# nyx-space/nyx

Measured on NVIDIA H100. Metric: trajectory-steps/sec (ensemble), higher is better.
Workload: dtype f64

## Files before the change

### nyx_b200/csrc/nyxb_tx.cu

```cuda
#include <algorithm>
#include <cmath>
#include <cstring>
#include <numeric>

#include "nyxb_tx.h"

#ifndef TX_MINB
#define TX_MINB 2
#endif

#ifndef NYXB_TX_TT
#define NYXB_TX_TT 1
#endif

namespace {
constexpr int TT = NYXB_TX_TT;
constexpr int NL = 32 * TT;
constexpr int HW = 3 * TT;
constexpr unsigned FULL = 0xffffffffu;

enum { TXF_H = 0, TXF_ERR, TXF_CR, TXF_CD, TXF_PM, TXF_DRY, TXF_EXTRA, TXF_SRPA, TXF_DRAGA, TXF_EVPREV, TXF_COUNT };
enum { TXI_EPOCH = 0, TXI_STEP, TXI_PREV_STEP, TXI_DET_STEP, TXI_NSTEPS, TXI_NREJ, TXI_NRHS, TXI_COUNT };
enum { TXW_FLAGS = 0, TXW_STATUS, TXW_RC, TXW_ATT, TXW_EVCNT, TXW_ACC, TXW_RCST, TXW_COUNT };
enum { F_FIXED = 1, F_PREVFIXED = 2, F_RETRY = 4, F_LAST = 8, F_DONE = 16, F_BACK = 32, F_VALID = 64 };

struct TxLayout {
    unsigned blob, ctx0, ctx_stride;
    unsigned wk, part, as, ysp, kst, nxt, er, ycur, rot, rn, f64, i64, i32;
    unsigned total;
};
__host__ __device__ inline TxLayout tx_layout(unsigned blob_bytes, int P, int N, int nctx) {
    (void)N;
    TxLayout L;
    L.blob = 0;
    L.ctx0 = (blob_bytes + 127u) & ~127u;
    unsigned o = 0;
    L.wk = o; o += 2u * (P == 16 ? 20u : 6u * (unsigned)P + 4u) * NL * 8;
    L.part = o; o += 2u * (unsigned)P * 4 * NL * 8;
    L.as = o; o += 2u * 18u * NL * 8;
    L.ysp = o; o += 2u * 3u * NL * 8;
    L.kst = o; o += NYXB_MAX_STAGES * 6 * NL * 8;
    L.nxt = o; o += 6 * NL * 8;
    L.er = o; o += 6 * NL * 8;
    L.ycur = o; o += 6 * NL * 8;
    L.rot = o; o += 6 * NL * 8;
    L.rn = o; o += 2u * 9u * NL * 8;
    L.f64 = o; o += TXF_COUNT * NL * 8;
    L.i64 = o; o += TXI_COUNT * NL * 8;
    L.i32 = o; o += TXW_COUNT * NL * 4;
    L.ctx_stride = (o + 127u) & ~127u;
    L.total = L.ctx0 + (unsigned)nctx * L.ctx_stride;
    return L;
}

struct TxSm {
    double *wk, *part, *as, *ysp, *kst, *nxt, *er, *ycur, *rot, *rn, *f64;
    long long* i64;
    int* i32;
};
__device__ __forceinline__ TxSm tx_views(unsigned char* smem, const TxLayout& L, int ctx, int N) {
    (void)N;
    unsigned char* b = smem + L.ctx0 + (unsigned)ctx * L.ctx_stride;
    TxSm sm;
    sm.wk = reinterpret_cast<double*>(b + L.wk); sm.part = reinterpret_cast<double*>(b + L.part);
    sm.as = reinterpret_cast<double*>(b + L.as); sm.ysp = reinterpret_cast<double*>(b + L.ysp);
    sm.kst = reinterpret_cast<double*>(b + L.kst); sm.nxt = reinterpret_cast<double*>(b + L.nxt);
    sm.er = reinterpret_cast<double*>(b + L.er); sm.ycur = reinterpret_cast<double*>(b + L.ycur);
    sm.rot = reinterpret_cast<double*>(b + L.rot); sm.rn = reinterpret_cast<double*>(b + L.rn);
    sm.f64 = reinterpret_cast<double*>(b + L.f64); sm.i64 = reinterpret_cast<long long*>(b + L.i64);
    sm.i32 = reinterpret_cast<int*>(b + L.i32);
    return sm;
}

__device__ __forceinline__ void nb_sync(int id, int count) { asm volatile("bar.sync %0, %1;" ::"r"(id), "r"(count) : "memory"); }
__device__ __forceinline__ void nb_arrive(int id, int count) { asm volatile("bar.arrive %0, %1;" ::"r"(id), "r"(count) : "memory"); }

__device__ __forceinline__ unsigned smem_u32(const void* p) { return (unsigned)__cvta_generic_to_shared(p); }
__device__ __forceinline__ void tx_mbar_init(unsigned long long* bar, unsigned count) {
    asm volatile("mbarrier.init.shared::cta.b64 [%0], %1;" ::"r"(smem_u32(bar)), "r"(count));
    asm volatile("fence.mbarrier_init.release.cluster;" ::: "memory");
}
__device__ __forceinline__ void tx_mbar_expect(unsigned long long* bar, unsigned bytes) {
    asm volatile("mbarrier.arrive.expect_tx.shared::cta.b64 _, [%0], %1;" ::"r"(smem_u32(bar)), "r"(bytes) : "memory");
}
__device__ __forceinline__ void tx_bulk_g2s(void* dst, const void* src, unsigned bytes, unsigned long long* bar) {
    asm volatile("cp.async.bulk.shared::cluster.global.mbarrier::complete_tx::bytes [%0], [%1], %2, [%3];"
                 ::"r"(smem_u32(dst)), "l"(src), "r"(bytes), "r"(smem_u32(bar)) : "memory");
}
__device__ __forceinline__ void tx_mbar_wait(unsigned long long* bar, unsigned parity) {
    asm volatile(
        "{\n"
        ".reg .pred p;\n"
        "TX_WAIT_LOOP:\n"
        "mbarrier.try_wait.parity.shared::cta.b64 p, [%0], %1;\n"
        "@p bra TX_WAIT_DONE;\n"
        "bra TX_WAIT_LOOP;\n"
        "TX_WAIT_DONE:\n"
        "}\n" ::"r"(smem_u32(bar)), "r"(parity) : "memory");
}

__device__ __forceinline__ void tx_mbar_arrive(unsigned long long* bar) {
// ... 273 lines not shown
        sm.i64[TXI_NSTEPS * NL + lane] = 0;
        sm.i64[TXI_NREJ * NL + lane] = 0;
        sm.i64[TXI_NRHS * NL + lane] = 0;
        sm.i32[TXW_FLAGS * NL + lane] = fl;
        sm.i32[TXW_STATUS * NL + lane] = 0;
        sm.i32[TXW_RC * NL + lane] = rc;
        sm.i32[TXW_ATT * NL + lane] = 1;
        sm.i32[TXW_EVCNT * NL + lane] = 0;
        sm.f64[TXF_EVPREV * NL + lane] = 0.0;
        if (sink.ev_kind)
            sm.f64[TXF_EVPREV * NL + lane] = event_eval(sink.ev_kind, sink.ev_value, state[tr], state[n + tr], state[2 * n + tr],
                                                        state[3 * n + tr], state[4 * n + tr], state[5 * n + tr]);
        if (valid && sink.cap > 0) sink.epoch[tr] = ep0;
    } else {
        const int pf = __ldcg(q.ws_flags + tr);
        const nyxb_details* dp = q.details + tr;
        sm.f64[TXF_CR * NL + lane] = __ldcg(out_state + 6 * n + tr);
        sm.f64[TXF_CD * NL + lane] = __ldcg(out_state + 7 * n + tr);
        sm.f64[TXF_PM * NL + lane] = __ldcg(out_state + 8 * n + tr);
        sm.f64[TXF_H * NL + lane] = __ldcg(q.ws_f64 + tr);
        sm.f64[TXF_EVPREV * NL + lane] = __ldcg(q.ws_f64 + n + tr);
        sm.f64[TXF_ERR * NL + lane] = __ldcg(&dp->error);
        sm.i64[TXI_EPOCH * NL + lane] = __ldcg(out_epoch + tr);
        const long long step_ns = __ldcg(q.ws_step + tr);
        sm.i64[TXI_STEP * NL + lane] = step_ns;
        sm.i64[TXI_PREV_STEP * NL + lane] = step_ns;
        sm.i64[TXI_DET_STEP * NL + lane] = __ldcg((const long long*)&dp->step_ns);
        sm.i64[TXI_NSTEPS * NL + lane] = __ldcg((const long long*)&dp->n_steps);
        sm.i64[TXI_NREJ * NL + lane] = __ldcg((const long long*)&dp->n_rejected);
        sm.i64[TXI_NRHS * NL + lane] = __ldcg((const long long*)&dp->n_rhs);
        sm.i32[TXW_ATT * NL + lane] = __ldcg(&dp->attempts);
        int fl = (pf & (F_FIXED | F_RETRY | F_DONE)) | (valid ? F_VALID : 0) | (duration < 0 ? F_BACK : 0);
        if (!valid) fl |= F_DONE;
        sm.i32[TXW_FLAGS * NL + lane] = fl;
        sm.i32[TXW_STATUS * NL + lane] = (pf & 8) ? NYXB_WARN_MAX_ATTEMPTS : 0;
        sm.i32[TXW_RC * NL + lane] = (pf >> 8) & 0xff;
        sm.i32[TXW_EVCNT * NL + lane] = sink.ev_kind ? __ldcg(sink.ev_crossings + tr) : 0;
    }
}

__device__ __noinline__ void tx_park_ctl(const DevSink& sink, const DevTxQueue& q, TxSm sm, int lane, size_t n, size_t tr,
                                         long long* step_io, double* out_state, long long* out_epoch, int* out_status) {
    const int fl = sm.i32[TXW_FLAGS * NL + lane];
    if (!(fl & F_VALID)) return;
    const int rc = sm.i32[TXW_RC * NL + lane], st = sm.i32[TXW_STATUS * NL + lane];
    out_state[6 * n + tr] = sm.f64[TXF_CR * NL + lane];
    out_state[7 * n + tr] = sm.f64[TXF_CD * NL + lane];
    out_state[8 * n + tr] = sm.f64[TXF_PM * NL + lane];
    out_epoch[tr] = sm.i64[TXI_EPOCH * NL + lane];
    const long long step_ns = sm.i64[TXI_STEP * NL + lane];
    q.ws_step[tr] = step_ns;
    q.ws_f64[tr] = sm.f64[TXF_H * NL + lane];
    q.ws_f64[n + tr] = sm.f64[TXF_EVPREV * NL + lane];
    q.ws_flags[tr] = (fl & (F_FIXED | F_RETRY | F_DONE)) | ((st & NYXB_WARN_MAX_ATTEMPTS) ? 8 : 0) | (rc << 8);
    nyxb_details d;
    d.step_ns = sm.i64[TXI_DET_STEP * NL + lane];
    d.error = sm.f64[TXF_ERR * NL + lane];
    d.attempts = sm.i32[TXW_ATT * NL + lane];
    d._pad = 0;
    d.n_steps = sm.i64[TXI_NSTEPS * NL + lane];
    d.n_rejected = sm.i64[TXI_NREJ * NL + lane];
    d.n_rhs = sm.i64[TXI_NRHS * NL + lane];
    q.details[tr] = d;
    int rc_out = rc;
    if (sink.ev_kind) {
        const int cnt = sm.i32[TXW_EVCNT * NL + lane];
        sink.ev_crossings[tr] = cnt;
        if (rc == 0 && cnt < sink.ev_trigger) rc_out = NYXB_ERR_EVENT_NOT_FOUND;
    }
    out_status[tr] = (st & NYXB_WARN_MAX_ATTEMPTS) | rc_out;
    if (step_io) step_io[tr] = step_ns;
    if (sink.cap > 0) sink.count[tr] = (d.n_steps + 1 < sink.cap) ? d.n_steps + 1 : sink.cap;
}

enum { AS_R = 0, AS_S = 9, AS_T, AS_U, AS_K0, AS_K1, AS_FAC, AS_P0, AS_P1, AS_P2, AS_COUNT };
enum { WK_UB = 0, WK_R2, WK_POW };
template <int P> struct TxWk {
    static constexpr bool ALL = (P != 16);
    static constexpr int E = 2 * P;
    static constexpr int COUNT = ALL ? WK_POW + 3 * E + 2 : WK_POW + 18;
    static constexpr int ZR = WK_POW, ZI = WK_POW + E + 1, RH = WK_POW + 2 * E + 1;
};

template <int P>
__device__ __forceinline__ void tx_prologue(const DevSetup& S, const TxSm& sm, int lane, int par, int j, const double* ysp, long long t_ns) {
    const DevGrav& gv = S.grav;
    const double* rn = sm.rn + par * 9 * NL + lane;
    const double p0 = ysp[lane], p1 = ysp[NL + lane], p2 = ysp[2 * NL + lane];
    double y0 = p0, y1 = p1, y2 = p2;
    double ir_c = 0.0;
    if (S.grav_body >= 0) {
        ir_c = rsqrt(fma(y2, y2, fma(y1, y1, y0 * y0)));
        tx_field_offset(S, t_ns, y0, y1, y2);
    }
    const double rb0 = fma(rn[2 * NL], y2, fma(rn[1 * NL], y1, rn[0] * y0));
    const double rb1 = fma(rn[5 * NL], y2, fma(rn[4 * NL], y1, rn[3 * NL] * y0));
    const double rb2 = fma(rn[8 * NL], y2, fma(rn[7 * NL], y1, rn[6 * NL] * y0));
    const double inv_r = rsqrt(fma(rb2, rb2, fma(rb1, rb1, rb0 * rb0)));
    if (S.grav_body < 0) ir_c = inv_r;
    const double rho = gv.r_eq * inv_r;
    const double s_ = rb0 * inv_r, t_ = rb1 * inv_r, u_ = rb2 * inv_r;
    double* wk = sm.wk + par * TxWk<P>::COUNT * NL + lane;
    if (j == 0) {
        wk[WK_UB * NL] = u_ * rho; wk[WK_R2 * NL] = rho * rho;
        double* as = sm.as + par * AS_COUNT * NL + lane;
#pragma unroll
        for (int k = 0; k < 9; ++k) as[(AS_R + k) * NL] = rn[k * NL];
        as[AS_S * NL] = s_; as[AS_T * NL] = t_; as[AS_U * NL] = u_;
        const double K0 = (gv.mu * gv.inv_r_eq) * inv_r;
        as[AS_K0 * NL] = K0; as[AS_K1 * NL] = K0 * rho;
        as[AS_FAC * NL] = -S.mu_central * ir_c * ir_c * ir_c;
        as[AS_P0 * NL] = p0; as[AS_P1 * NL] = p1; as[AS_P2 * NL] = p2;
        if constexpr (!TxWk<P>::ALL) {
            double zr = s_, zi = t_, rp = rho;
#pragma unroll
            for (int k = 0; k < 6; ++k) {
                wk[(WK_POW + 3 * k) * NL] = zr; wk[(WK_POW + 3 * k + 1) * NL] = zi; wk[(WK_POW + 3 * k + 2) * NL] = rp;
                const double nr = fma(zr, zr, -(zi * zi));
                zi = 2.0 * zr * zi; zr = nr; rp *= rp;
            }
        }
    } else if constexpr (TxWk<P>::ALL) {
        constexpr int E = TxWk<P>::E;
        static_assert(E > 8 && E <= 24, "published powers");
        double* wr = wk + TxWk<P>::ZR * NL;
        double* wi = wk + TxWk<P>::ZI * NL;
        double zr[9], zi[9];
        zr[1] = s_; zi[1] = t_;
#pragma unroll
        for (int lo = 1; lo < 8; lo *= 2) {
#pragma unroll
            for (int k = 1; k <= lo; ++k) {
                zr[lo + k] = fma(zr[lo], zr[k], -(zi[lo] * zi[k]));
                zi[lo + k] = fma(zr[lo], zi[k], zi[lo] * zr[k]);
            }
        }
        if (j == 1) {
            wr[0] = 1.0; wi[0] = 0.0;
#pragma unroll
            for (int k = 1; k <= 8; ++k) { wr[k * NL] = zr[k]; wi[k * NL] = zi[k]; }
            double rp[9];
            rp[1] = rho;
#pragma unroll
            for (int lo = 1; lo < 8; lo *= 2) {
#pragma unroll
                for (int k = 1; k <= lo; ++k) rp[lo + k] = rp[lo] * rp[k];
            }
            double* wp = wk + TxWk<P>::RH * NL;
            const double r16 = rp[8] * rp[8];
#pragma unroll
            for (int k = 1; k <= 8; ++k) {
                wp[k * NL] = rp[k];
                if (8 + k <= E) wp[(8 + k) * NL] = (k == 8) ? r16 : rp[8] * rp[k];
                if (16 + k <= E) wp[(16 + k) * NL] = r16 * rp[k];
            }
        } else {
            const double z16r = fma(zr[8], zr[8], -(zi[8] * zi[8])), z16i = 2.0 * zr[8] * zi[8];
#pragma unroll
            for (int k = 1; k <= 8; ++k) {
                if (8 + k <= E) {
                    wr[(8 + k) * NL] = (k == 8) ? z16r : fma(zr[8], zr[k], -(zi[8] * zi[k]));
                    wi[(8 + k) * NL] = (k == 8) ? z16i : fma(zr[8], zi[k], zi[8] * zr[k]);
                }
                if (16 + k <= E) {
                    wr[(16 + k) * NL] = fma(z16r, zr[k], -(z16i * zi[k]));
                    wi[(16 + k) * NL] = fma(z16r, zi[k], z16i * zr[k]);
                }
            }
        }
    }
}

struct TxRotBase { double sa, ca, sd, cd, sw, cw; };
__device__ __forceinline__ void tx_dcm(const DevRotation& rot, const TxRotBase& b, long long off_ns, double (&R)[9]) {
    if (rot.kind == 0) {
        R[0] = 1; R[1] = 0; R[2] = 0; R[3] = 0; R[4] = 1; R[5] = 0; R[6] = 0; R[7] = 0; R[8] = 1;
        return;
    }
    const double dt_s = (double)off_ns * 1e-9;
    const double da = rot.ra_dot * dt_s, dd = rot.dec_dot * dt_s, dw = rot.wdot * dt_s;
    const double sa = fma(b.ca, da, b.sa), ca = fma(-b.sa, da, b.ca);
    const double sd = fma(b.cd, dd, b.sd), cd = fma(-b.sd, dd, b.cd);
    double sdl, cdl;
    if (fabs(dw) < 0.02) {
        const double z = dw * dw;
        sdl = dw * fma(z, fma(z, 1.0 / 120.0, -1.0 / 6.0), 1.0);
        cdl = fma(z, fma(z, fma(z, -1.0 / 720.0, 1.0 / 24.0), -0.5), 1.0);
    } else {
        det_sincos(dw, sdl, cdl);
    }
    const double sw = fma(b.sw, cdl, b.cw * sdl), cw = fma(b.cw, cdl, -(b.sw * sdl));
    const double b00 = -sa, b01 = ca;
    const double b10 = -(sd * ca), b11 = -(sd * sa), b12 = cd;
    R[0] = fma(cw, b00, sw * b10); R[1] = fma(cw, b01, sw * b11); R[2] = sw * b12;
    R[3] = fma(cw, b10, -(sw * b00)); R[4] = fma(cw, b11, -(sw * b01)); R[5] = cw * b12;
    R[6] = cd * ca; R[7] = cd * sa; R[8] = sd;
}

__device__ __forceinline__ TxRotBase tx_rot_base(const DevRotation& rot, long long epoch) {
    TxRotBase b;
    const double t_s = dur_to_seconds(epoch);
    const double d = t_s / 86400.0;
    const double Tc = d / 36525.0;
    det_sincos((rot.ra0 + rot.ra1 * Tc) * NYXB_DEG2RAD, b.sa, b.ca);
    det_sincos((rot.dec0 + rot.dec1 * Tc) * NYXB_DEG2RAD, b.sd, b.cd);
    det_sincos(fmod(rot.w0 + rot.w1 * d, 360.0) * NYXB_DEG2RAD, b.sw, b.cw);
    return b;
}
__device__ __forceinline__ void tx_rot_store(double* rot, int lane, const TxRotBase& b) {
    rot[lane] = b.sa; rot[NL + lane] = b.ca; rot[2 * NL + lane] = b.sd; rot[3 * NL + lane] = b.cd; rot[4 * NL + lane] = b.sw;
    rot[5 * NL + lane] = b.cw;
}

template <int W, int NB>
__device__ __forceinline__ void tx_start_powers(const double* wk, double& zar, double& zai, double& pa, double& zbr, double& zbi, double& pb) {
    const double rho = wk[(WK_POW + 2) * NL];
    bool fa = true, fb = true;
    zar = 1.0; zai = 0.0; zbr = 1.0; zbi = 0.0; pa = rho; pb = rho;
#pragma unroll
    for (int k = 0; k < NB; ++k) {
        const double br = wk[(WK_POW + 3 * k) * NL], bi = wk[(WK_POW + 3 * k + 1) * NL], bp = wk[(WK_POW + 3 * k + 2) * NL];
        if ((W >> k) & 1) {
            if (fa) { zar = br; zai = bi; fa = false; }
            else { const double nr = fma(zar, br, -(zai * bi)); zai = fma(zar, bi, zai * br); zar = nr; }
            pa *= bp;
        } else {
            if (fb) { zbr = br; zbi = bi; fb = false; }
            else { const double nr = fma(zbr, br, -(zbi * bi)); zbi = fma(zbr, bi, zbi * br); zbr = nr; }
            pb *= bp;
        }
    }
}

template <int P, int NCTX>
__global__ void __launch_bounds__((P + HW * NCTX) * 32, 1)
nyxb_k_tx(const __grid_constant__ DevSetup S, const __grid_constant__ DevTx Tx, const __grid_constant__ DevTxQueue q, size_t n,
          const double* __restrict__ state, const double* __restrict__ consts, const long long* __restrict__ epoch0,
          long long end_epoch, long long* step_io, double* out_state, long long* out_epoch, int* out_status, const DevSink sink,
          unsigned blob_bytes, unsigned off_recK, unsigned off_seed, unsigned off_sched) {
    static_assert(P <= NYXB_TX_MAXP && NCTX >= 1 && NCTX <= 2, "walker positions / set contexts");
    extern __shared__ __align__(128) unsigned char smem[];
    __shared__ __align__(8) unsigned long long tma_bar;
    __shared__ __align__(8) unsigned long long ready_bar[NCTX][2];
    __shared__ int s_set[NCTX], s_fresh[NCTX], s_exit[NCTX], s_done_half[NCTX][TT], s_slice_end[NCTX];
    __shared__ __align__(8) unsigned long long kick_bar;
    const int tid = threadIdx.x, lane = tid & 31, w = tid >> 5;
#ifdef NYXB_TX_TRACE
    int tr_n = 0;
#endif
    constexpr int NPOW = 6;
    static_assert(P == 8 || P == 10 || P == 16, "walker positions");
    static_assert(TT == 1 || NCTX == 1, "sets of 64 trajectories: one set context per CTA");
    constexpr int NT_RW = (P + HW) * 32;
    constexpr int NT_HB = HW * 32;
    constexpr int BAR_PER_CTX = 5;
    const int N = S.grav.N;
    const int stages = S.tb.stages;
    const TxLayout L = tx_layout(blob_bytes, P, N, NCTX);
    const double2* recA = reinterpret_cast<const double2*>(smem + L.blob);
    const double* recK = reinterpret_cast<const double*>(smem + L.blob + off_recK);
    const double* colseed = reinterpret_cast<const double*>(smem + L.blob + off_seed);
    const int* sched = reinterpret_cast<const int*>(smem + L.blob + off_sched);

    if (tid == 0) {
        tx_mbar_init(&tma_bar, 1);
#pragma unroll
        tx_mbar_init(&kick_bar, 1);
#pragma unroll
        for (int c = 0; c < NCTX; ++c) {
            s_exit[c] = 0;
            tx_mbar_init(&ready_bar[c][0], NT_HB);
            tx_mbar_init(&ready_bar[c][1], NT_HB);
        }
    }
    __syncthreads();
    if (tid == 0) {
        tx_mbar_expect(&tma_bar, blob_bytes);
        tx_bulk_g2s(smem + L.blob, Tx.recA, blob_bytes, &tma_bar);
    }
    tx_mbar_wait(&tma_bar, 0);
    __syncthreads();

    if (w < P) {
        const int pos = (P == 8) ? ((0x23571046u >> (4 * w)) & 0xfu) : w;
        const int* my = sched + pos * (2 + 2 * Tx.kmax);
        const int rec_off = my[0], ncol = my[1];
        unsigned active = (1u << NCTX) - 1u;
        unsigned phases = 0;
        const unsigned ready0 = smem_u32(&ready_bar[0][0]);
        int stage0 = 0, stage1 = 0, pref = 0;
        while (active) {
            {
                int c = -1, par = 0;
                TX_TRACE(TR_POLL, 0, 0);
                for (;;) {
#pragma unroll
                    for (int k = 0; k < NCTX; ++k) {
                        const int cc = (pref + k) % NCTX;
                        if (c >= 0 || !((active >> cc) & 1u)) continue;
                        const int pp = (cc == 0 ? stage0 : stage1) & 1;
                        const bool ok = tx_mbar_test(ready0 + 8u * (unsigned)(2 * cc + pp), (phases >> (2 * cc + pp)) & 1u);
                        if (__all_sync(FULL, ok)) { c = cc; par = pp; }
                    }
                    if (c >= 0) break;
                    __nanosleep(20);
                }
                phases ^= 1u << (2 * c + par);
                const int st = (c == 0) ? stage0 : stage1;
                if (st == 0 && *(volatile int*)&s_exit[c]) { active &= ~(1u << c); continue; }
                const int stn = (st + 1 == stages) ? 0 : st + 1;
                if (c == 0) stage0 = stn; else stage1 = stn;
                pref = (c + 1) % NCTX;
                TX_TRACE(TR_WALK, c, st);
                const TxSm sm = tx_views(smem, L, c, N);
                TxLaneState t[TT];
#pragma unroll
                for (int u = 0; u < TT; ++u) {
                    const double* wk = sm.wk + par * TxWk<P>::COUNT * NL + u * 32 + lane;
                    t[u].ub = wk[WK_UB * NL]; t[u].r2 = wk[WK_R2 * NL];
                    t[u].dc = t[u].ub + t[u].ub; t[u].dg = t[u].r2 + t[u].r2;
                    if constexpr (TxWk<P>::ALL) {
                        constexpr int E = TxWk<P>::E;
                        t[u].zar = wk[(TxWk<P>::ZR + pos) * NL]; t[u].zai = wk[(TxWk<P>::ZI + pos) * NL];
                        t[u].pa = wk[(TxWk<P>::RH + pos + 1) * NL];
                        t[u].zbr = wk[(TxWk<P>::ZR + E - 1 - pos) * NL]; t[u].zbi = wk[(TxWk<P>::ZI + E - 1 - pos) * NL];
                        t[u].pb = wk[(TxWk<P>::RH + E - pos) * NL];
                        t[u].qr = wk[(TxWk<P>::ZR + E) * NL]; t[u].qi = wk[(TxWk<P>::ZI + E) * NL]; t[u].qp = wk[(TxWk<P>::RH + E) * NL];
                    } else {
                        switch (pos) {
#define NYXB_TX_CASE(WW) case WW: tx_start_powers<WW, NPOW - 1>(wk, t[u].zar, t[u].zai, t[u].pa, t[u].zbr, t[u].zbi, t[u].pb); break;
                            NYXB_TX_CASE(0) NYXB_TX_CASE(1) NYXB_TX_CASE(2) NYXB_TX_CASE(3) NYXB_TX_CASE(4) NYXB_TX_CASE(5) NYXB_TX_CASE(6) NYXB_TX_CASE(7)
                            NYXB_TX_CASE(8) NYXB_TX_CASE(9) NYXB_TX_CASE(10) NYXB_TX_CASE(11) NYXB_TX_CASE(12) NYXB_TX_CASE(13) NYXB_TX_CASE(14)
                            default: tx_start_powers<15, NPOW - 1>(wk, t[u].zar, t[u].zai, t[u].pa, t[u].zbr, t[u].zbi, t[u].pb); break;
#undef NYXB_TX_CASE
                        }
                        t[u].qr = wk[(WK_POW + 3 * (NPOW - 1)) * NL]; t[u].qi = wk[(WK_POW + 3 * (NPOW - 1) + 1) * NL];
                        t[u].qp = wk[(WK_POW + 3 * (NPOW - 1) + 2) * NL];
                    }
                    t[u].X = 0.0; t[u].Y = 0.0; t[u].Z = 0.0; t[u].W = 0.0;
                }
                const double2* A = recA + 2 * rec_off;
                const double* K = recK + rec_off;
                double2 a01 = A[0], a23 = A[1];
                double kk = K[0];
                int len = my[3];
                {
                    const double4 sd = *reinterpret_cast<const double4*>(colseed + 4 * my[2]);
#pragma unroll
                    for (int u = 0; u < TT; ++u) {
                        t[u].cQ = t[u].pa * sd.x; t[u].cc1 = sd.w * t[u].ub; t[u].cg = sd.w * t[u].r2;
                        t[u].cS5 = t[u].cQ * sd.y; t[u].cS6 = t[u].cQ * sd.z;
                    }
                }
                for (int k = 0; k < ncol; k += 2) {
                    {
                        const int len_n = my[5 + 2 * k];
                        const double4 sd_n = *reinterpret_cast<const double4*>(colseed + 4 * my[4 + 2 * k]);
                        tx_column<false>(A, K, a01, a23, kk, len, t);
#pragma unroll
                        for (int u = 0; u < TT; ++u) {
                            t[u].cQ = t[u].pb * sd_n.x; t[u].cc1 = sd_n.w * t[u].ub; t[u].cg = sd_n.w * t[u].r2;
                            t[u].cS5 = t[u].cQ * sd_n.y; t[u].cS6 = t[u].cQ * sd_n.z;
                            const double nr = fma(t[u].zar, t[u].qr, -(t[u].zai * t[u].qi));
                            t[u].zai = fma(t[u].zar, t[u].qi, t[u].zai * t[u].qr); t[u].zar = nr; t[u].pa *= t[u].qp;
                        }
                        len = len_n;
                    }
                    if (k + 1 >= ncol) break;
                    {
                        const int len_n = my[7 + 2 * k];
                        const double4 sd_n = *reinterpret_cast<const double4*>(colseed + 4 * my[6 + 2 * k]);
                        tx_column<true>(A, K, a01, a23, kk, len, t);
#pragma unroll
                        for (int u = 0; u < TT; ++u) {
                            t[u].cQ = t[u].pa * sd_n.x; t[u].cc1 = sd_n.w * t[u].ub; t[u].cg = sd_n.w * t[u].r2;
                            t[u].cS5 = t[u].cQ * sd_n.y; t[u].cS6 = t[u].cQ * sd_n.z;
                            const double nr = fma(t[u].zbr, t[u].qr, -(t[u].zbi * t[u].qi));
                            t[u].zbi = fma(t[u].zbr, t[u].qi, t[u].zbi * t[u].qr); t[u].zbr = nr; t[u].pb *= t[u].qp;
                        }
                        len = len_n;
                    }
                }
#pragma unroll
                for (int u = 0; u < TT; ++u) {
                    double* pt = sm.part + ((par * P + pos) * 4) * NL + u * 32 + lane;
                    pt[0] = t[u].X; pt[NL] = t[u].Y; pt[2 * NL] = t[u].Z; pt[3 * NL] = t[u].W;
                }
                nb_arrive(1 + c * BAR_PER_CTX + 3 + par, NT_RW);
                TX_TRACE(TR_WALK_END, c, st);
            }
        }
        return;
    }

    const int c = (w - P) / HW, j = ((w - P) % HW) % 3, half = ((w - P) % HW) / 3;
    const int tl = half * 32 + lane;
    const TxSm sm = tx_views(smem, L, c, N);
    const int BAR_HB = 1 + c * BAR_PER_CTX, BAR_DONE = BAR_HB + 3;
    const DevGrav& gv = S.grav;
    const bool has_extra = S.n_bodies > 0 || S.has_srp || S.has_drag || S.n_xgrav > 0;
    const bool lead = (j == 0);
    const bool lead0 = lead && half == 0;
    auto set_done = [&]() {
        bool d = s_done_half[c][0] != 0;
        if (TT == 2) d = d && s_done_half[c][TT - 1] != 0;
        return d;
    };
    const double* ta = S.tb.a;

    bool kick_pending = (NCTX > 1 && c == 0);
    if (NCTX > 1 && c == 1) {
        if (lead0 && lane == 0) tx_mbar_wait(&kick_bar, 0);
        nb_sync(BAR_HB, NT_HB);
    }

    for (;;) {
        if (lead0 && lane == 0) {
            int set = -1, fresh = 0;
            if (atomicAdd(q.ctl + TXQ_FRESH, 0) < q.n_sets) {
                const int f = atomicAdd(q.ctl + TXQ_FRESH, 1);
                if (f < q.n_sets) { set = f; fresh = 1; }
            }
            if (set < 0 && q.slice > 0) {
                while (atomicCAS(q.ctl + TXQ_LOCK, 0, 1) != 0) __nanosleep(64);
                __threadfence();
                volatile int* vc = q.ctl;
                const int head = vc[TXQ_HEAD], tail = vc[TXQ_TAIL];
                if (head < tail) {
                    set = ((volatile int*)q.ring)[head % q.n_sets];
                    vc[TXQ_HEAD] = head + 1;
                }
                __threadfence();
                atomicExch(q.ctl + TXQ_LOCK, 0);
            }
            s_set[c] = set; s_fresh[c] = fresh;
            s_exit[c] = set < 0;
        }
        nb_sync(BAR_HB, NT_HB);
        if (s_exit[c] && kick_pending && lead0 && lane == 0) tx_mbar_arrive(&kick_bar);
        if (s_exit[c]) {
            tx_mbar_arrive(&ready_bar[c][0]);
            return;
        }
        const int set = s_set[c];
        const int round = s_fresh[c] ? 0 : 1;
        const size_t traj_raw = (size_t)set * NL + tl;
        const bool valid = traj_raw < n;
        const size_t tr = valid ? traj_raw : (size_t)set * NL;

#pragma unroll
        for (int hh = 0; hh < 2; ++hh) {
            const int cc = j + 3 * hh;
            const double yc = (round == 0) ? state[(size_t)cc * n + tr] : __ldcg(out_state + (size_t)cc * n + tr);
            sm.ycur[cc * NL + tl] = yc;
            if (round == 0 && valid && sink.cap > 0) sink.state[((size_t)cc * sink.cap) * n + tr] = yc;
        }
        if (lead) {
            tx_load_ctl(S, sink, q, sm, tl, n, tr, valid, round, state, consts, epoch0, end_epoch, step_io, out_state, out_epoch);
            tx_pick_step(sm, tl, end_epoch);
            const bool done = sm.i32[TXW_FLAGS * NL + tl] & F_DONE;
            const bool all = __all_sync(FULL, done);
            if (lane == 0) { s_done_half[c][half] = all; if (half == 0) s_slice_end[c] = 0; }
            if (gv.rot.kind != 0) tx_rot_store(sm.rot, tl, tx_rot_base(gv.rot, sm.i64[TXI_EPOCH * NL + tl]));
        }
        nb_sync(BAR_HB, NT_HB);

        for (int it = 0; !set_done(); ++it) {
            TX_TRACE(TR_TOP, c, 0);
            const double h = sm.f64[TXF_H * NL + tl];
            const long long epoch = sm.i64[TXI_EPOCH * NL + tl];
            const double r_own = sm.ycur[j * NL + tl], v_own = sm.ycur[(3 + j) * NL + tl];
            TxRotBase rb_;
            rb_.sa = 0.0; rb_.ca = 1.0; rb_.sd = 1.0; rb_.cd = 0.0; rb_.sw = 0.0; rb_.cw = 1.0;
            TxRotBase rb_next = rb_;
            const bool fixed = sm.i32[TXW_FLAGS * NL + tl] & F_FIXED;
            double nx_r = r_own, nx_v = v_own, er_r = 0.0, er_v = 0.0;
            int rc_acc = 0;
            double Rn[9];
            sm.kst[(0 * 6 + j) * NL + tl] = v_own;
            sm.ysp[(0 * 3 + j) * NL + tl] = r_own;
            const long long off1 = (stages > 1) ? dur_from_seconds(S.tb.c[0] * h) : 0;
            if (stages > 1) sm.ysp[(1 * 3 + j) * NL + tl] = fma(h, ta[0] * v_own, r_own);
            nb_sync(BAR_HB, NT_HB);
            TX_TRACE(TR_PRIMED, c, 0);
            if (lead) {
                if (gv.rot.kind != 0) {
                    rb_.sa = sm.rot[tl]; rb_.ca = sm.rot[NL + tl]; rb_.sd = sm.rot[2 * NL + tl]; rb_.cd = sm.rot[3 * NL + tl];
                    rb_.sw = sm.rot[4 * NL + tl]; rb_.cw = sm.rot[5 * NL + tl];
                }
                tx_dcm(gv.rot, rb_, 0, Rn);
#pragma unroll
                for (int k = 0; k < 9; ++k) sm.rn[k * NL + tl] = Rn[k];
            } else if (j == 1 && stages > 1) {
                TxRotBase rb1 = rb_;
                if (gv.rot.kind != 0) {
                    rb1.sa = sm.rot[tl]; rb1.ca = sm.rot[NL + tl]; rb1.sd = sm.rot[2 * NL + tl]; rb1.cd = sm.rot[3 * NL + tl];
                    rb1.sw = sm.rot[4 * NL + tl]; rb1.cw = sm.rot[5 * NL + tl];
                }
                tx_dcm(gv.rot, rb1, off1, Rn);
#pragma unroll
                for (int k = 0; k < 9; ++k) sm.rn[(9 + k) * NL + tl] = Rn[k];
            }
            nb_sync(BAR_HB, NT_HB);
            TX_TRACE(TR_DCM01, c, 0);
            tx_prologue<P>(S, sm, tl, 0, j, sm.ysp, epoch);
            tx_mbar_arrive(&ready_bar[c][0]);
            TX_TRACE(TR_READY, c, 0);
            if (stages > 1) {
                tx_prologue<P>(S, sm, tl, 1, j, sm.ysp + 3 * NL, epoch + off1);
                tx_mbar_arrive(&ready_bar[c][1]);
                TX_TRACE(TR_READY, c, 1);
            }
            nb_sync(BAR_HB, NT_HB);
            for (int i = 0; i < stages; ++i) {
                const int par = i & 1;
                double preV = 0.0, preP = 0.0;
                long long off2 = 0;
                {
                    const double vi = sm.kst[(i * 6 + j) * NL + tl];
                    if (!fixed) er_r = fma(h * S.tb.e[i], vi, er_r);
                    nx_r = fma(h * S.tb.b[i], vi, nx_r);
                }
                if (j == 1 && i == 0 && gv.rot.kind != 0)
                    rb_next = tx_rot_base(gv.rot, epoch + (fixed ? sm.i64[TXI_STEP * NL + tl] : dur_from_seconds(h)));
                if (i + 1 < stages) {
                    const double* arow = ta + i * NYXB_MAX_STAGES;
                    const double* kc = sm.kst + (3 + j) * NL + tl;
                    double w0 = 0.0, w1 = 0.0;
                    int l = 0;
                    for (; l + 1 < i; l += 2) { w0 = fma(arow[l], kc[l * 6 * NL], w0); w1 = fma(arow[l + 1], kc[(l + 1) * 6 * NL], w1); }
                    if (l < i) w0 = fma(arow[l], kc[l * 6 * NL], w0);
                    preV = w0 + w1;
                }
                if (i + 2 < stages) {
                    const double* arow = ta + (i + 1) * NYXB_MAX_STAGES;
                    const double* kc = sm.kst + j * NL + tl;
                    double w0 = 0.0, w1 = 0.0;
                    int m = 0;
                    for (; m + 1 <= i; m += 2) { w0 = fma(arow[m], kc[m * 6 * NL], w0); w1 = fma(arow[m + 1], kc[(m + 1) * 6 * NL], w1); }
                    if (m <= i) w0 = fma(arow[m], kc[m * 6 * NL], w0);
                    preP = w0 + w1;
                    off2 = dur_from_seconds(S.tb.c[i + 1] * h);
                    TX_TRACE(TR_PRE_DONE, c, i);
                    if (lead) {
                        tx_dcm(gv.rot, rb_, off2, Rn);
#pragma unroll
                        for (int k = 0; k < 9; ++k) sm.rn[(par * 9 + k) * NL + tl] = Rn[k];
                    }
                }
                TX_TRACE(TR_DCM_DONE, c, i);
                if (kick_pending && i == stages / 2) {
                    if (lead0 && lane == 0) tx_mbar_arrive(&kick_bar);
                    kick_pending = false;
                }
                TX_TRACE(TR_DONE_WAIT, c, i);
                nb_sync(BAR_DONE + par, NT_RW);
                TX_TRACE(TR_DONE_SEEN, c, i);

                double X, Y, Z, Wt;
                {
                    double ax[4] = {0.0, 0.0, 0.0, 0.0}, ay[4] = {0.0, 0.0, 0.0, 0.0}, az[4] = {0.0, 0.0, 0.0, 0.0}, aw4[4] = {0.0, 0.0, 0.0, 0.0};
#pragma unroll
                    for (int p = 0; p < P; ++p) {
                        const double* pt = sm.part + ((par * P + p) * 4) * NL + tl;
                        ax[p & 3] += pt[0]; ay[p & 3] += pt[NL]; az[p & 3] += pt[2 * NL]; aw4[p & 3] += pt[3 * NL];
                    }
                    X = (ax[0] + ax[1]) + (ax[2] + ax[3]); Y = (ay[0] + ay[1]) + (ay[2] + ay[3]);
                    Z = (az[0] + az[1]) + (az[2] + az[3]); Wt = (aw4[0] + aw4[1]) + (aw4[2] + aw4[3]);
                }
                TX_TRACE(TR_REDUCED, c, i);
                const double* as = sm.as + par * AS_COUNT * NL + tl;
                const double K0 = as[AS_K0 * NL], K1 = as[AS_K1 * NL];
                const double aw = -K0 * Wt;
                const double ab0 = fma(aw, as[AS_S * NL], K1 * X), ab1 = fma(aw, as[AS_T * NL], K1 * Y), ab2 = fma(aw, as[AS_U * NL], K1 * Z);
                double acc = fma(as[AS_FAC * NL], as[(AS_P0 + j) * NL],
                                 fma(as[(AS_R + 6 + j) * NL], ab2, fma(as[(AS_R + 3 + j) * NL], ab1, as[(AS_R + j) * NL] * ab0)));
                if (has_extra) {
                    double yy[9], aa[3] = {0.0, 0.0, 0.0};
                    const double hz = (i > 0) ? h * 0.0 : 0.0;
                    yy[0] = as[AS_P0 * NL]; yy[1] = as[AS_P1 * NL]; yy[2] = as[AS_P2 * NL];
#pragma unroll
                    for (int e = 0; e < 3; ++e) yy[3 + e] = sm.kst[(i * 6 + e) * NL + tl];
                    yy[6] = sm.f64[TXF_CR * NL + tl] + hz; yy[7] = sm.f64[TXF_CD * NL + tl] + hz; yy[8] = sm.f64[TXF_PM * NL + tl] + hz;
                    const long long offi = (i > 0) ? dur_from_seconds(S.tb.c[i - 1] * h) : 0;
                    const int rcx = tx_extra(S, sm.f64[TXF_DRY * NL + tl], sm.f64[TXF_EXTRA * NL + tl], sm.f64[TXF_SRPA * NL + tl],
                                             sm.f64[TXF_DRAGA * NL + tl], epoch + offi, yy, aa);
                    acc += (j == 0) ? aa[0] : (j == 1 ? aa[1] : aa[2]);
                    if (rcx && !rc_acc) rc_acc = rcx | ((i + 1) << 8);
                }
                sm.kst[(i * 6 + 3 + j) * NL + tl] = acc;
                if (!fixed) er_v = fma(h * S.tb.e[i], acc, er_v);
                nx_v = fma(h * S.tb.b[i], acc, nx_v);
                if (i + 1 < stages) {
                    const double vn = fma(h, fma(ta[i * NYXB_MAX_STAGES + i], acc, preV), v_own);
                    sm.kst[((i + 1) * 6 + j) * NL + tl] = vn;
                    if (i + 2 < stages)
                        sm.ysp[(par * 3 + j) * NL + tl] = fma(h, fma(ta[(i + 1) * NYXB_MAX_STAGES + i + 1], vn, preP), r_own);
                    TX_TRACE(TR_ACC_DONE, c, i);
                    nb_sync(BAR_HB, NT_HB);
                    TX_TRACE(TR_HB_PASSED, c, i);
                    if (i + 2 < stages) {
                        tx_prologue<P>(S, sm, tl, par, j, sm.ysp + par * 3 * NL, epoch + off2);
                        tx_mbar_arrive(&ready_bar[c][par]);
                        TX_TRACE(TR_READY, c, i + 2);
                    }
                }
            }
            TX_TRACE(TR_STAGES_END, c, 0);
            sm.nxt[j * NL + tl] = nx_r; sm.nxt[(3 + j) * NL + tl] = nx_v;
            sm.er[j * NL + tl] = er_r; sm.er[(3 + j) * NL + tl] = er_v;
            if (lead) sm.i32[TXW_RCST * NL + tl] = rc_acc;
            nb_sync(BAR_HB, NT_HB);
            TX_TRACE(TR_CTRL_IN, c, 0);
            if (lead) {
                tx_controller(S, sink, sm, tl, n, tr, stages);
                TX_TRACE(TR_CTRL_OUT, c, 0);
                const bool slice_end = q.slice > 0 && it + 1 >= q.slice;
                if (!slice_end) tx_pick_step(sm, tl, end_epoch);
                TX_TRACE(TR_PICKED, c, 0);
                const bool done = sm.i32[TXW_FLAGS * NL + tl] & F_DONE;
                const bool all = __all_sync(FULL, done);
                if (lane == 0) { s_done_half[c][half] = all; if (half == 0) s_slice_end[c] = slice_end; }
            }
            nb_sync(BAR_HB, NT_HB);
            TX_TRACE(TR_CTRL_END, c, 0);
            if (sm.i32[TXW_ACC * NL + tl]) {
                if (j == 1 && gv.rot.kind != 0) tx_rot_store(sm.rot, tl, rb_next);
                const long long ns = sm.i64[TXI_NSTEPS * NL + tl];
#pragma unroll
                for (int hh = 0; hh < 2; ++hh) {
                    const int cc = j + 3 * hh;
                    const double nx = sm.nxt[cc * NL + tl];
                    sm.ycur[cc * NL + tl] = nx;
                    if (valid && ns < sink.cap) sink.state[((size_t)cc * sink.cap + (size_t)ns) * n + tr] = nx;
                }
            }
            TX_TRACE(TR_COMMITTED, c, 0);
            if (s_slice_end[c]) break;
        }

        if (kick_pending) {
            if (lead0 && lane == 0) tx_mbar_arrive(&kick_bar);
            kick_pending = false;
        }
        if (valid) {
            out_state[(size_t)j * n + tr] = sm.ycur[j * NL + tl];
            out_state[(size_t)(j + 3) * n + tr] = sm.ycur[(j + 3) * NL + tl];
        }
        if (lead) tx_park_ctl(sink, q, sm, tl, n, tr, step_io, out_state, out_epoch, out_status);
        __threadfence();
        nb_sync(BAR_HB, NT_HB);
        if (lead0 && lane == 0 && !set_done()) {
            while (atomicCAS(q.ctl + TXQ_LOCK, 0, 1) != 0) __nanosleep(64);
            __threadfence();
            volatile int* vc = q.ctl;
            const int tail = vc[TXQ_TAIL];
            ((volatile int*)q.ring)[tail % q.n_sets] = set;
            vc[TXQ_TAIL] = tail + 1;
            __threadfence();
            atomicExch(q.ctl + TXQ_LOCK, 0);
        }
        nb_sync(BAR_HB, NT_HB);
    }
}

template <int P, int NCTX>
cudaError_t tx_launch_p(const DevSetup* S, const DevTx* Tx, const DevTxQueue* q, size_t n, const double* state, const double* consts,
                        const long long* epoch0, long long end_epoch, long long* step_io, double* out_state, long long* out_epoch,
                        int* out_status, const DevSink* sink, int grid, size_t smem, unsigned blob_bytes, unsigned off_recK,
                        unsigned off_seed, unsigned off_sched, cudaStream_t stream) {
    cudaError_t e = cudaFuncSetAttribute(nyxb_k_tx<P, NCTX>, cudaFuncAttributeMaxDynamicSharedMemorySize, (int)smem);
    if (e != cudaSuccess) return e;
    nyxb_k_tx<P, NCTX><<<grid, (P + HW * NCTX) * 32, smem, stream>>>(*S, *Tx, *q, n, state, consts, epoch0, end_epoch, step_io, out_state,
                                                                  out_epoch, out_status, *sink, blob_bytes, off_recK, off_seed, off_sched);
    return cudaGetLastError();
}

struct TxBlob { unsigned off_recK, off_seed, off_sched, bytes; };
TxBlob tx_blob(int N, int P, int n_rec, int kmax) {
    TxBlob b;
    unsigned o = (unsigned)(n_rec + 1) * 32u;
    b.off_recK = o; o += (((unsigned)(n_rec + 2) + 1u) & ~1u) * 8u;
    b.off_seed = o; o += (unsigned)(N + 2) * 32u;
    b.off_sched = o; o += (unsigned)P * (2u + 2u * (unsigned)kmax) * 4u;
    b.bytes = (o + 15u) & ~15u;
    return b;
}
}

#if NYXB_TX_TT == 1
void nyxb_tx_build_host(int N, int M, const double* c_nm, const double* s_nm, int P, TxHost& out) {
    const double sqrt2 = std::sqrt(2.0);
    auto C = [&](int n, int m) { return (n <= N && m <= M && m <= n) ? c_nm[(size_t)n * (N + 1) + m] : 0.0; };
    auto Sx = [&](int n, int m) { return (n <= N && m <= M && m <= n) ? s_nm[(size_t)n * (N + 1) + m] : 0.0; };
    auto vr01 = [&](int n, int m) {
        double nf = n, mf = m;
        double v = std::sqrt((nf - mf) * (nf + mf + 1.0));
        return m == 0 ? v / sqrt2 : v;
    };
    auto vr11 = [&](int n, int m) {
        double nf = n, mf = m;
        double v = std::sqrt(((2.0 * nf + 1.0) * (nf + mf + 2.0) * (nf + mf + 1.0)) / (2.0 * nf + 3.0));
        return m == 0 ? v / sqrt2 : v;
    };
    auto scale = [&](int n, int m) -> long double {
        long double adiag = 1.0L, dfact = 1.0L;
        for (int k = 1; k <= m; ++k) { adiag *= sqrtl(1.0L + 1.0L / (2.0L * k)); dfact *= (2.0L * k - 1.0L); }
        long double g = adiag / dfact;
        for (int k = m + 1; k <= n; ++k) g *= sqrtl(((2.0L * k + 1.0L) * (k - m)) / ((2.0L * k - 1.0L) * (k + m)));
        for (int k = 2; k <= n - m; ++k) g /= (long double)k;
        return g;
    };
    const int mcols = std::min(M + 1, N + 1);
    auto col_len = [&](int m) { return (std::max(N + 1 - m, 1) + 1) & ~1; };
    std::vector<std::vector<int>> cols(P);
    for (int m = 1; m <= mcols; ++m) {
        const int r = (m - 1) % (2 * P);
        cols[r < P ? r : 2 * P - 1 - r].push_back(m);
    }
    out.P = P;
    out.kmax = 1;
    for (auto& cl : cols) out.kmax = std::max(out.kmax, (int)cl.size());
    out.kmax += 1;
    out.n_rec = 0;
    for (int m = 1; m <= mcols; ++m) out.n_rec += col_len(m);
    out.recA.assign((size_t)(out.n_rec + 1) * 4, 0.0);
    out.recK.assign((size_t)(out.n_rec + 2), 0.0);
    out.colseed.assign((size_t)(N + 2) * 4, 0.0);
    out.sched.assign((size_t)P * (2 + 2 * out.kmax), 0);
    for (int m = 1; m <= mcols; ++m) {
        long double dfact = 1.0L;
        for (int k = 1; k <= m; ++k) dfact *= (2.0L * k - 1.0L);
        double* s = &out.colseed[(size_t)m * 4];
        s[0] = (double)dfact;
        if (m >= 2) {
            long double f = (long double)sqrt2 * vr11(m - 1, m - 1) * scale(m, m);
            s[1] = (double)(f * C(m - 1, m - 1));
            s[2] = (double)(f * Sx(m - 1, m - 1));
        }
        s[3] = 2.0 * m + 1.0;
    }
    int e = 0;
    for (int w = 0; w < P; ++w) {
        int* sc = &out.sched[(size_t)w * (2 + 2 * out.kmax)];
        sc[0] = e;
        sc[1] = (int)cols[w].size();
        for (size_t k = 0; k < cols[w].size(); ++k) {
            const int m = cols[w][k];
            sc[2 + 2 * k] = m;
            sc[3 + 2 * k] = col_len(m);
            auto kappa = [&](int n) -> double {
                return (double)(((long double)vr11(n - 1, m - 1) * scale(n, m)) / ((long double)vr01(n - 1, m - 1) * scale(n - 1, m)));
            };
            for (int n = m; n < m + col_len(m); ++n, ++e) {
                if (n > N) continue;
                const long double sc_ = scale(n, m);
// ... 69 lines not shown
```

Before: 132.8 million.

## Add dedicated rotor warp per context for DCM rotation work when P=8, NCTX=2

For the P=8, two-context configuration, each set context gets an extra helper warp (a 'rotor') that computes the rotation DCMs, the next rotation base and publishes the rotation matrix into the shared stage area. This takes that work off the lead and j==1 helper warps' critical path. Helper role assignment is rotated per context and the walker position permutation changes to match. It adds one warp per context, which raises the per-CTA thread count and named-barrier participant counts and may add synchronization overhead.

After: 134.7 million (median of 6 runs). 1.01x the previous value.

```diff
diff --git a/nyx_b200/csrc/nyxb_tx.cu b/nyx_b200/csrc/nyxb_tx.cu
--- a/nyx_b200/csrc/nyxb_tx.cu
+++ b/nyx_b200/csrc/nyxb_tx.cu
@@ -16,7 +16,8 @@
 namespace {
 constexpr int TT = NYXB_TX_TT;
 constexpr int NL = 32 * TT;
-constexpr int HW = 3 * TT;
+constexpr int HC = 3 * TT;
+__host__ __device__ constexpr int tx_helpers(int P, int nctx) { return HC + ((P == 8 && nctx == 2) ? 1 : 0); }
 constexpr unsigned FULL = 0xffffffffu;
 
 enum { TXF_H = 0, TXF_ERR, TXF_CR, TXF_CD, TXF_PM, TXF_DRY, TXF_EXTRA, TXF_SRPA, TXF_DRAGA, TXF_EVPREV, TXF_COUNT };
@@ -456,7 +457,7 @@
     static constexpr int ZR = WK_POW, ZI = WK_POW + E + 1, RH = WK_POW + 2 * E + 1;
 };
 
-template <int P>
+template <int P, bool ROT>
 __device__ __forceinline__ void tx_prologue(const DevSetup& S, const TxSm& sm, int lane, int par, int j, const double* ysp, long long t_ns) {
     const DevGrav& gv = S.grav;
     const double* rn = sm.rn + par * 9 * NL + lane;
@@ -478,8 +479,10 @@
     if (j == 0) {
         wk[WK_UB * NL] = u_ * rho; wk[WK_R2 * NL] = rho * rho;
         double* as = sm.as + par * AS_COUNT * NL + lane;
-#pragma unroll
-        for (int k = 0; k < 9; ++k) as[(AS_R + k) * NL] = rn[k * NL];
+        if constexpr (!ROT) {
+#pragma unroll
+            for (int k = 0; k < 9; ++k) as[(AS_R + k) * NL] = rn[k * NL];
+        }
         as[AS_S * NL] = s_; as[AS_T * NL] = t_; as[AS_U * NL] = u_;
         const double K0 = (gv.mu * gv.inv_r_eq) * inv_r;
         as[AS_K0 * NL] = K0; as[AS_K1 * NL] = K0 * rho;
@@ -543,6 +546,13 @@
             }
         }
     }
+}
+
+__device__ __forceinline__ void tx_rot_publish(const TxSm& sm, int lane, int par) {
+    const double* rn = sm.rn + par * 9 * NL + lane;
+    double* as = sm.as + par * AS_COUNT * NL + lane;
+#pragma unroll
+    for (int k = 0; k < 9; ++k) as[(AS_R + k) * NL] = rn[k * NL];
 }
 
 struct TxRotBase { double sa, ca, sd, cd, sw, cw; };
@@ -607,7 +617,7 @@
 }
 
 template <int P, int NCTX>
-__global__ void __launch_bounds__((P + HW * NCTX) * 32, 1)
+__global__ void __launch_bounds__((P + tx_helpers(P, NCTX) * NCTX) * 32, 1)
 nyxb_k_tx(const __grid_constant__ DevSetup S, const __grid_constant__ DevTx Tx, const __grid_constant__ DevTxQueue q, size_t n,
           const double* __restrict__ state, const double* __restrict__ consts, const long long* __restrict__ epoch0,
           long long end_epoch, long long* step_io, double* out_state, long long* out_epoch, int* out_status, const DevSink sink,
@@ -625,7 +635,9 @@
     constexpr int NPOW = 6;
     static_assert(P == 8 || P == 10 || P == 16, "walker positions");
     static_assert(TT == 1 || NCTX == 1, "sets of 64 trajectories: one set context per CTA");
-    constexpr int NT_RW = (P + HW) * 32;
+    constexpr int HW = tx_helpers(P, NCTX);
+    constexpr bool ROT = HW > HC;
+    constexpr int NT_RW = (P + HC) * 32;
     constexpr int NT_HB = HW * 32;
     constexpr int BAR_PER_CTX = 5;
     const int N = S.grav.N;
@@ -656,7 +668,7 @@
     __syncthreads();
 
     if (w < P) {
-        const int pos = (P == 8) ? ((0x23571046u >> (4 * w)) & 0xfu) : w;
+        const int pos = (P != 8) ? w : ((((ROT ? 0x54762301u : 0x23571046u) >> (4 * w)) & 0xfu));
         const int* my = sched + pos * (2 + 2 * Tx.kmax);
         const int rec_off = my[0], ncol = my[1];
         unsigned active = (1u << NCTX) - 1u;
@@ -767,13 +779,16 @@
         return;
     }
 
-    const int c = (w - P) / HW, j = ((w - P) % HW) % 3, half = ((w - P) % HW) / 3;
+    const int c = (w - P) / HW;
+    const int role = ROT ? ((w - P) % HW + 2 * c) % HW : (w - P) % HW;
+    const bool rotor = ROT && role == HC;
+    const int j = rotor ? 0 : role % 3, half = rotor ? 0 : role / 3;
     const int tl = half * 32 + lane;
     const TxSm sm = tx_views(smem, L, c, N);
     const int BAR_HB = 1 + c * BAR_PER_CTX, BAR_DONE = BAR_HB + 3;
     const DevGrav& gv = S.grav;
     const bool has_extra = S.n_bodies > 0 || S.has_srp || S.has_drag || S.n_xgrav > 0;
-    const bool lead = (j == 0);
+    const bool lead = !rotor && j == 0;
     const bool lead0 = lead && half == 0;
     auto set_done = [&]() {
         bool d = s_done_half[c][0] != 0;
@@ -822,12 +837,14 @@
         const bool valid = traj_raw < n;
         const size_t tr = valid ? traj_raw : (size_t)set * NL;
 
-#pragma unroll
-        for (int hh = 0; hh < 2; ++hh) {
-            const int cc = j + 3 * hh;
-            const double yc = (round == 0) ? state[(size_t)cc * n + tr] : __ldcg(out_state + (size_t)cc * n + tr);
-            sm.ycur[cc * NL + tl] = yc;
-            if (round == 0 && valid && sink.cap > 0) sink.state[((size_t)cc * sink.cap) * n + tr] = yc;
+        if (!rotor) {
+#pragma unroll
+            for (int hh = 0; hh < 2; ++hh) {
+                const int cc = j + 3 * hh;
+                const double yc = (round == 0) ? state[(size_t)cc * n + tr] : __ldcg(out_state + (size_t)cc * n + tr);
+                sm.ycur[cc * NL + tl] = yc;
+                if (round == 0 && valid && sink.cap > 0) sink.state[((size_t)cc * sink.cap) * n + tr] = yc;
+            }
         }
         if (lead) {
             tx_load_ctl(S, sink, q, sm, tl, n, tr, valid, round, state, consts, epoch0, end_epoch, step_io, out_state, out_epoch);
@@ -839,11 +856,72 @@
         }
         nb_sync(BAR_HB, NT_HB);
 
-        for (int it = 0; !set_done(); ++it) {
+        if (rotor) {
+            for (int it = 0; !set_done(); ++it) {
+                TX_TRACE(TR_TOP, c, 0);
+                const double h = sm.f64[TXF_H * NL + tl];
+                const long long epoch = sm.i64[TXI_EPOCH * NL + tl];
+                const bool fixed = sm.i32[TXW_FLAGS * NL + tl] & F_FIXED;
+                TxRotBase rb_;
+                rb_.sa = 0.0; rb_.ca = 1.0; rb_.sd = 1.0; rb_.cd = 0.0; rb_.sw = 0.0; rb_.cw = 1.0;
+                if (gv.rot.kind != 0) {
+                    rb_.sa = sm.rot[tl]; rb_.ca = sm.rot[NL + tl]; rb_.sd = sm.rot[2 * NL + tl]; rb_.cd = sm.rot[3 * NL + tl];
+                    rb_.sw = sm.rot[4 * NL + tl]; rb_.cw = sm.rot[5 * NL + tl];
+                }
+                TxRotBase rb_next = rb_;
+                double Rn[9];
+                nb_sync(BAR_HB, NT_HB);
+                TX_TRACE(TR_PRIMED, c, 0);
+                tx_dcm(gv.rot, rb_, 0, Rn);
+#pragma unroll
+                for (int k = 0; k < 9; ++k) sm.rn[k * NL + tl] = Rn[k];
+                nb_sync(BAR_HB, NT_HB);
+                TX_TRACE(TR_DCM01, c, 0);
+                tx_rot_publish(sm, tl, 0);
+                tx_mbar_arrive(&ready_bar[c][0]);
+                TX_TRACE(TR_READY, c, 0);
+                if (stages > 1) {
+                    tx_rot_publish(sm, tl, 1);
+                    tx_mbar_arrive(&ready_bar[c][1]);
+                    TX_TRACE(TR_READY, c, 1);
+                }
+                nb_sync(BAR_HB, NT_HB);
+                for (int i = 0; i < stages; ++i) {
+                    const int par = i & 1;
+                    if (i + 2 < stages) {
+                        tx_dcm(gv.rot, rb_, dur_from_seconds(S.tb.c[i + 1] * h), Rn);
+#pragma unroll
+                        for (int k = 0; k < 9; ++k) sm.rn[(par * 9 + k) * NL + tl] = Rn[k];
+                    }
+                    TX_TRACE(TR_DCM_DONE, c, i);
+                    if (i == 0 && gv.rot.kind != 0)
+                        rb_next = tx_rot_base(gv.rot, epoch + (fixed ? sm.i64[TXI_STEP * NL + tl] : dur_from_seconds(h)));
+                    if (i + 1 < stages) {
+                        nb_sync(BAR_HB, NT_HB);
+                        if (i + 2 < stages) {
+                            tx_rot_publish(sm, tl, par);
+                            tx_mbar_arrive(&ready_bar[c][par]);
+                            TX_TRACE(TR_READY, c, i + 2);
+                        }
+                    }
+                }
+                TX_TRACE(TR_STAGES_END, c, 0);
+                nb_sync(BAR_HB, NT_HB);
+                nb_sync(BAR_HB, NT_HB);
+                TX_TRACE(TR_CTRL_END, c, 0);
+                if (gv.rot.kind != 0 && sm.i32[TXW_ACC * NL + tl]) tx_rot_store(sm.rot, tl, rb_next);
+                TX_TRACE(TR_COMMITTED, c, 0);
+                if (s_slice_end[c]) break;
+            }
+        }
+
+        for (int it = 0; !rotor && !set_done(); ++it) {
             TX_TRACE(TR_TOP, c, 0);
             const double h = sm.f64[TXF_H * NL + tl];
             const long long epoch = sm.i64[TXI_EPOCH * NL + tl];
             const double r_own = sm.ycur[j * NL + tl], v_own = sm.ycur[(3 + j) * NL + tl];
+            const bool dcm_helper = !ROT && lead;
+            const bool rbn_helper = !ROT && j == 1;
             TxRotBase rb_;
             rb_.sa = 0.0; rb_.ca = 1.0; rb_.sd = 1.0; rb_.cd = 0.0; rb_.sw = 0.0; rb_.cw = 1.0;
             TxRotBase rb_next = rb_;
@@ -857,7 +935,7 @@
             if (stages > 1) sm.ysp[(1 * 3 + j) * NL + tl] = fma(h, ta[0] * v_own, r_own);
             nb_sync(BAR_HB, NT_HB);
             TX_TRACE(TR_PRIMED, c, 0);
-            if (lead) {
+            if (dcm_helper) {
                 if (gv.rot.kind != 0) {
                     rb_.sa = sm.rot[tl]; rb_.ca = sm.rot[NL + tl]; rb_.sd = sm.rot[2 * NL + tl]; rb_.cd = sm.rot[3 * NL + tl];
                     rb_.sw = sm.rot[4 * NL + tl]; rb_.cw = sm.rot[5 * NL + tl];
@@ -877,11 +955,11 @@
             }
             nb_sync(BAR_HB, NT_HB);
             TX_TRACE(TR_DCM01, c, 0);
-            tx_prologue<P>(S, sm, tl, 0, j, sm.ysp, epoch);
+            tx_prologue<P, ROT>(S, sm, tl, 0, j, sm.ysp, epoch);
             tx_mbar_arrive(&ready_bar[c][0]);
             TX_TRACE(TR_READY, c, 0);
             if (stages > 1) {
-                tx_prologue<P>(S, sm, tl, 1, j, sm.ysp + 3 * NL, epoch + off1);
+                tx_prologue<P, ROT>(S, sm, tl, 1, j, sm.ysp + 3 * NL, epoch + off1);
                 tx_mbar_arrive(&ready_bar[c][1]);
                 TX_TRACE(TR_READY, c, 1);
             }
@@ -895,7 +973,7 @@
                     if (!fixed) er_r = fma(h * S.tb.e[i], vi, er_r);
                     nx_r = fma(h * S.tb.b[i], vi, nx_r);
                 }
-                if (j == 1 && i == 0 && gv.rot.kind != 0)
+                if (rbn_helper && i == 0 && gv.rot.kind != 0)
                     rb_next = tx_rot_base(gv.rot, epoch + (fixed ? sm.i64[TXI_STEP * NL + tl] : dur_from_seconds(h)));
                 if (i + 1 < stages) {
                     const double* arow = ta + i * NYXB_MAX_STAGES;
@@ -916,7 +994,7 @@
                     preP = w0 + w1;
                     off2 = dur_from_seconds(S.tb.c[i + 1] * h);
                     TX_TRACE(TR_PRE_DONE, c, i);
-                    if (lead) {
+                    if (dcm_helper) {
                         tx_dcm(gv.rot, rb_, off2, Rn);
 #pragma unroll
                         for (int k = 0; k < 9; ++k) sm.rn[(par * 9 + k) * NL + tl] = Rn[k];
@@ -974,7 +1052,7 @@
                     nb_sync(BAR_HB, NT_HB);
                     TX_TRACE(TR_HB_PASSED, c, i);
                     if (i + 2 < stages) {
-                        tx_prologue<P>(S, sm, tl, par, j, sm.ysp + par * 3 * NL, epoch + off2);
+                        tx_prologue<P, ROT>(S, sm, tl, par, j, sm.ysp + par * 3 * NL, epoch + off2);
                         tx_mbar_arrive(&ready_bar[c][par]);
                         TX_TRACE(TR_READY, c, i + 2);
                     }
@@ -999,7 +1077,7 @@
             nb_sync(BAR_HB, NT_HB);
             TX_TRACE(TR_CTRL_END, c, 0);
             if (sm.i32[TXW_ACC * NL + tl]) {
-                if (j == 1 && gv.rot.kind != 0) tx_rot_store(sm.rot, tl, rb_next);
+                if (rbn_helper && gv.rot.kind != 0) tx_rot_store(sm.rot, tl, rb_next);
                 const long long ns = sm.i64[TXI_NSTEPS * NL + tl];
 #pragma unroll
                 for (int hh = 0; hh < 2; ++hh) {
@@ -1017,7 +1095,7 @@
             if (lead0 && lane == 0) tx_mbar_arrive(&kick_bar);
             kick_pending = false;
         }
-        if (valid) {
+        if (valid && !rotor) {
             out_state[(size_t)j * n + tr] = sm.ycur[j * NL + tl];
             out_state[(size_t)(j + 3) * n + tr] = sm.ycur[(j + 3) * NL + tl];
         }
@@ -1045,7 +1123,7 @@
                         unsigned off_seed, unsigned off_sched, cudaStream_t stream) {
     cudaError_t e = cudaFuncSetAttribute(nyxb_k_tx<P, NCTX>, cudaFuncAttributeMaxDynamicSharedMemorySize, (int)smem);
     if (e != cudaSuccess) return e;
-    nyxb_k_tx<P, NCTX><<<grid, (P + HW * NCTX) * 32, smem, stream>>>(*S, *Tx, *q, n, state, consts, epoch0, end_epoch, step_io, out_state,
+    nyxb_k_tx<P, NCTX><<<grid, (P + tx_helpers(P, NCTX) * NCTX) * 32, smem, stream>>>(*S, *Tx, *q, n, state, consts, epoch0, end_epoch, step_io, out_state,
                                                                   out_epoch, out_status, *sink, blob_bytes, off_recK, off_seed, off_sched);
     return cudaGetLastError();
 }
```
